# nanoporetech/pomfret

Hardware: AMD Instinct MI355X
Metric: aligned reads/sec (methphase kernel) (higher is better)
Workload: dtype u32/f32

## Files before the change

### pomfret_amd/csrc/pf_load.hip

```cpp
#include <hip/hip_runtime.h>
#include <stdint.h>
#include "pf_device.h"
#include "pf_load.h"

#define DEV static __device__ __forceinline__
#define NT_C 2u
#ifndef PF_K0_SEQ_REREAD
#define PF_K0_SEQ_REREAD 0
#endif

#ifdef PF_K0_PROFILE
DEV unsigned long long k0_now() {
    unsigned long long t;
    __builtin_amdgcn_sched_barrier(0);
    asm volatile("s_memtime %0\n\ts_waitcnt lgkmcnt(0)" : "=s"(t) :: "memory");
    __builtin_amdgcn_sched_barrier(0);
    return t;
}
#define K0_STAMP(i) do { const unsigned long long t_ = k0_now(); \
    if (d->ctr && lane == 0) atomicAdd(&d->ctr[8 + (i)], t_ - k0_t); k0_t = t_; } while (0)
#define K0_T0 unsigned long long k0_t = k0_now()
#else
#define K0_STAMP(i) do { } while (0)
#define K0_T0 do { } while (0)
#endif
#define NT_G 4u
#ifndef PF_K0_NOINL
#define PF_K0_NOINL 0
#endif
#if PF_K0_NOINL & 1
#define DEV_HBM static __device__ __attribute__((noinline))
#else
#define DEV_HBM DEV
#endif
#if PF_K0_NOINL & 2
#define DEV_COLD static __device__ __attribute__((noinline))
#else
#define DEV_COLD DEV
#endif
#ifndef PF_K0_PLACE
#define PF_K0_PLACE 1
#endif
#ifndef PF_K0_WALK2
#define PF_K0_WALK2 1
#endif
#ifndef PF_K0_FUSEC
#define PF_K0_FUSEC 1
#endif
#ifndef PF_K0_PADFIX
#define PF_K0_PADFIX 1
#endif
#ifndef PF_K0_NBRARE
#define PF_K0_NBRARE 1
#endif
#ifndef PF_K0_RANKDPP
#define PF_K0_RANKDPP 1
#endif
#ifndef PF_K0_HDRFAST
#define PF_K0_HDRFAST 1
#endif
#ifndef PF_K0_EMITDPP
#define PF_K0_EMITDPP 1
#endif
#ifndef PF_K0_ROWSKIP
#define PF_K0_ROWSKIP 1
#endif
#ifndef PF_K0_TILE128
#define PF_K0_TILE128 1
#endif
#ifndef PF_K0_DIAG1
#define PF_K0_DIAG1 0
#endif
#if PF_K0_DIAG1
#define K0_DIAG1(d) ((d)->diag == 1u)
#else
#define K0_DIAG1(d) false
#endif
#ifndef PF_K0_WPE
#define PF_K0_WPE 8
#endif

DEV uint32_t uni(uint32_t x) { return (uint32_t)__builtin_amdgcn_readfirstlane((int)x); }
DEV uint64_t lanemask_lt(uint32_t lane) { return lane ? (~0ull >> (64 - lane)) : 0ull; }
DEV uint32_t popc(uint64_t m) { return (uint32_t)__popcll(m); }
DEV uint32_t below_cnt(uint64_t b) {
    return __builtin_amdgcn_mbcnt_hi((uint32_t)(b >> 32), __builtin_amdgcn_mbcnt_lo((uint32_t)b, 0u));
}
DEV uint32_t rdl(uint32_t x, uint32_t l) { return (uint32_t)__builtin_amdgcn_readlane((int)x, (int)l); }

#define K0_CONST __attribute__((address_space(4)))
typedef const K0_CONST pf_load_dev *K0Args;
typedef const K0_CONST pf_k0_hdr *K0HdrP;
DEV K0Args k0_args() { return (K0Args)__builtin_amdgcn_kernarg_segment_ptr(); }
template <typename P>
DEV P k0_late(P p) {
    asm volatile("" : "+s"(p));
    return p;
}

DEV void wsync() {
    __builtin_amdgcn_fence(__ATOMIC_RELEASE, "workgroup");
    __builtin_amdgcn_wave_barrier();
    __builtin_amdgcn_fence(__ATOMIC_ACQUIRE, "workgroup");
}

DEV uint32_t dpp_shr_add(uint32_t x, const int ctrl) {
    uint32_t y;
    switch (ctrl) {
    case 1: y = (uint32_t)__builtin_amdgcn_update_dpp(0, (int)x, 0x111, 0xF, 0xF, true); break;
    case 2: y = (uint32_t)__builtin_amdgcn_update_dpp(0, (int)x, 0x112, 0xF, 0xF, true); break;
    case 4: y = (uint32_t)__builtin_amdgcn_update_dpp(0, (int)x, 0x114, 0xF, 0xF, true); break;
    case 8: y = (uint32_t)__builtin_amdgcn_update_dpp(0, (int)x, 0x118, 0xF, 0xF, true); break;
    case 15: y = (uint32_t)__builtin_amdgcn_update_dpp(0, (int)x, 0x142, 0xA, 0xF, false); break;
    default: y = (uint32_t)__builtin_amdgcn_update_dpp(0, (int)x, 0x143, 0xC, 0xF, false); break;
    }
    return x + y;
}
DEV uint32_t wscan(uint32_t x, uint32_t) {
    x = dpp_shr_add(x, 1);
    x = dpp_shr_add(x, 2);
    x = dpp_shr_add(x, 4);
    x = dpp_shr_add(x, 8);
    x = dpp_shr_add(x, 15);
    x = dpp_shr_add(x, 31);
    return x;
}
DEV uint64_t wscan64(uint64_t x, uint32_t lane) {
#pragma unroll
    for (int o = 1; o < 64; o <<= 1) {
        const uint64_t y = __shfl_up(x, o, 64);
        if (lane >= (uint32_t)o) x += y;
    }
    return x;
}
DEV uint64_t rdl64(uint64_t x, uint32_t l) {
    return ((uint64_t)rdl((uint32_t)(x >> 32), l) << 32) | rdl((uint32_t)x, l);
}

DEV uint32_t nib(const uint8_t *s, uint32_t i) { return (s[i >> 1] >> ((~i & 1u) << 2)) & 0xFu; }
DEV uint32_t nibw(uint64_t w, uint32_t i) { return (uint32_t)(w >> (8u * (i >> 1) + ((i & 1u) ? 0u : 4u))) & 0xFu; }
DEV uint32_t match16(uint64_t w, uint32_t tb, uint32_t nv) {
    uint32_t m = 0;
#pragma unroll
    for (uint32_t i = 0; i < 16; i++) m |= (nibw(w, i) == tb && i < nv) ? (1u << i) : 0u;
    return m;
}
DEV uint32_t select_bit(uint32_t m, uint32_t k) {
    for (uint32_t i = 0; i < k; i++) m &= m - 1;
    return (uint32_t)__builtin_ctz(m);
}
DEV bool is_digit(uint32_t c) { return c >= '0' && c <= '9'; }
// ... 17 lines not shown
    uint8_t eC[PF_K0_EC];
    uint8_t mC[2 * PF_K0_EC];
};
struct K0Seq {
    uint16_t sb[8 * 64];
    uint8_t sc[8 * 64];
};
struct K0Wide {
    uint32_t E[128], Off[128];
    uint32_t gE[16], sE[4];
    uint8_t T[128];
    uint32_t mV[64];
    uint8_t mC[64];
};
struct K0W {
    uint32_t T[PF_K0_TCAP];
    union {
        struct {
            uint32_t opE[64], opOff[64], opA[64];
            uint8_t opT[64];
            union {
                K0Seq s;
                K0Merge mg;
            } u;
        };
        K0Wide w;
    };
};
static_assert(sizeof(K0W) == 5120, "K0W: 5 KB per wave, 20,480 B per block");

struct K0Out {
    uint32_t n, first, last;
    uint32_t sorted, lim;
    uint32_t *pos;
    uint8_t *cat;
};

struct K0Tgt { uint32_t nd, nc, mi, th, te; uint64_t ml; };
#define PF_K0_MAXT 8
#define PF_K0_TW 7
struct K0Tgts { K0Tgt t0; uint32_t n, over; uint32_t *xt; };
DEV void k0_tgt_put(uint32_t *xt, uint32_t e, const K0Tgt &t, uint32_t lane) {
    if (lane == 0) {
        uint32_t *q = xt + PF_K0_TW * (e - 1);
        q[0] = t.nd; q[1] = t.nc; q[2] = t.mi; q[3] = t.th; q[4] = t.te; q[5] = (uint32_t)t.ml;
        q[6] = (uint32_t)(t.ml >> 32);
    }
}
DEV K0Tgt k0_tgt_get(const K0Tgts &T, uint32_t e) {
    if (e == 0) return T.t0;
    const uint32_t *q = T.xt + PF_K0_TW * (e - 1);
    K0Tgt t;
    t.nd = q[0]; t.nc = q[1]; t.mi = q[2]; t.th = q[3]; t.te = q[4];
    t.ml = ((uint64_t)q[6] << 32) | q[5];
    return t;
}

DEV uint32_t bytes_eq(uint32_t w, uint32_t c) {
    const uint32_t t = w ^ (c * 0x01010101u);
    return ~(((t & 0x7F7F7F7Fu) + 0x7F7F7F7Fu) | t) & 0x80808080u;
}
DEV uint32_t bytes_in(int32_t b, uint32_t lo, uint32_t hi) {
    const int32_t s = min(max((int32_t)lo - b, 0), 4), e = min(max((int32_t)hi - b, 0), 4);
    const uint32_t ml = s >= 4 ? 0u : 0x80808080u << (8 * s);
    const uint32_t mh = e <= 0 ? 0u : 0x80808080u >> (8 * (4 - e));
    return ml & mh;
}
DEV uint32_t wsum_small(uint32_t c) {
    return popc(__ballot(c & 1u)) + 2u * popc(__ballot(c & 2u)) + 4u * popc(__ballot(c & 4u));
}
DEV uint64_t nondigit_bytes(uint64_t y) {
    const uint64_t hi = (y & 0xF0F0F0F0F0F0F0F0ull) ^ 0x3030303030303030ull;
    const uint64_t hz = ~(((hi & 0x7F7F7F7F7F7F7F7Full) + 0x7F7F7F7F7F7F7F7Full) | hi) & 0x8080808080808080ull;
    const uint64_t ge10 = ((y & 0x0F0F0F0F0F0F0F0Full) + 0x7676767676767676ull) & 0x8080808080808080ull;
    return (~hz & 0x8080808080808080ull) | ge10;
}
DEV uint32_t swar_dec(uint64_t y, uint32_t n) {
    uint64_t z = (y & ((1ull << (8 * n)) - 1)) << (8 * (8 - n));
    z = ((z & 0x0F0F0F0F0F0F0F0Full) * 2561u) >> 8;
    z = ((z & 0x00FF00FF00FF00FFull) * 6553601u) >> 16;
    return (uint32_t)(((z & 0x0000FFFF0000FFFFull) * 42949672960001ull) >> 32);
}

struct K0Hdr { uint32_t base, strand, nc, h; int mi; };

template <bool MULTI>
DEV bool k0_mm_entries(const uint32_t *gw, const uint8_t *mm, uint32_t mis, uint32_t mlen, uint32_t mln,
                       uint32_t lane, K0Tgts &T) {
    T.n = 0;
    T.over = 0;
    T.t0.nd = 0;
    if (mlen == 0) return true;
    const uint32_t wend = mis + mlen;
    const uint32_t kmaxw = (wend - 1) / 4 + 1;
    auto ld = [&](uint32_t k) { return gw[min(k, kmaxw)]; };
    uint32_t k0 = 0;
    uint32_t w = ld(lane), pw = ld(64 + lane), pw2 = ld(128 + lane), pw3 = ld(192 + lane);
    auto byte_at = [&](uint32_t x) -> uint32_t {
        const uint32_t kx = (mis + x) >> 2, sh = 8 * ((mis + x) & 3u);
        if (kx - k0 < 64) return (rdl(w, kx - k0) >> sh) & 0xFFu;
        if (kx - k0 < 128) return (rdl(pw, kx - k0 - 64) >> sh) & 0xFFu;
        return mm[x];
    };
    K0Hdr H;
#if PF_K0_HDRFAST
    auto dword_at = [&](uint32_t kx) -> uint32_t {
        if (kx - k0 < 64) return rdl(w, kx - k0);
        if (kx - k0 < 128) return rdl(pw, kx - k0 - 64);
        return gw[min(kx, kmaxw)];
    };
#endif
    auto header = [&](uint32_t i) {
#if PF_K0_HDRFAST
        if (i + 3 < mlen) {
            const uint32_t x = mis + i, kx = x >> 2, sh = 8u * (x & 3u);
            const uint32_t lo = dword_at(kx);
            const uint32_t b4 = sh ? (lo >> sh) | (dword_at(kx + 1) << (32u - sh)) : lo;
            const uint32_t c2 = (b4 >> 16) & 0xFFu, c3 = b4 >> 24;
            if (is_alpha(c2) && !is_alpha(c3)) {
                H.base = b4 & 0xFFu;
                H.strand = (b4 >> 8) & 0xFFu;
                H.nc = 1;
                H.mi = c2 == 'm' ? 0 : -1;
                H.h = i + 3 + ((c3 == '.' || c3 == '?') ? 1u : 0u);
                return;
            }
        }
#endif
        H.base = byte_at(i);
        H.strand = i + 1 < mlen ? byte_at(i + 1) : 0u;
        uint32_t h = i + 2, nc = 0;
        int mi = -1;
        uint32_t c = h < mlen ? byte_at(h) : 0u;
        if (is_digit(c)) {
            while (h < mlen && is_digit(byte_at(h))) h++;
            nc = 1;
        } else {
            while (h < mlen && is_alpha(c = byte_at(h))) {
                if (c == 'm' && mi < 0) mi = (int)nc;
                nc++;
                h++;
            }
        }
        if (h < mlen && ((c = byte_at(h)) == '.' || c == '?')) h++;
        H.h = h; H.nc = nc; H.mi = mi;
    };
    uint64_t ml_cur = 0;
    auto close = [&](uint32_t i, uint32_t e, uint32_t commas) -> bool {
        if (e - i < 3) return false;
        if (H.strand != '+' && H.strand != '-') return false;
        if (H.nc == 0) return false;
        if (H.base == ',') commas--;
        if (H.base == 'C' && H.mi >= 0 && commas > 0) {
            if (mln && ml_cur + (uint64_t)commas * H.nc > mln) return false;
            if (!MULTI && T.n) { T.n = 2; return true; }
            if (T.n == PF_K0_MAXT) { T.over = 1; return true; }
            K0Tgt t;
            t.nd = commas; t.nc = H.nc; t.mi = (uint32_t)H.mi; t.th = H.h; t.te = e; t.ml = ml_cur;
            if (T.n == 0) T.t0 = t;
            else if constexpr (MULTI) k0_tgt_put(T.xt, T.n, t, lane);
            T.n++;
        }
        ml_cur += (uint64_t)commas * H.nc;
        return true;
    };
    uint32_t i = 0, ci = 0, cg = 0;
    header(0);
    for (;;) {
        const int32_t b = (int32_t)(4 * (k0 + lane)) - (int32_t)mis;
        const uint32_t vm = bytes_in(b, 0, mlen);
        const uint32_t sm = bytes_eq(w, ';') & vm, cm = bytes_eq(w, ',') & vm;
        const uint32_t ncl = (uint32_t)__builtin_popcount(cm);
        const uint32_t cin = wscan(ncl, lane);
        for (uint64_t bs = __ballot(sm != 0); bs; bs &= bs - 1) {
            const uint32_t l0 = (uint32_t)__ffsll((long long)bs) - 1;
            const uint32_t sml = rdl(sm, l0), cml = rdl(cm, l0), cb0 = cg + rdl(cin, l0) - rdl(ncl, l0);
            for (uint32_t m = sml; m; m &= m - 1) {
                const uint32_t sb = (uint32_t)__builtin_ctz(m) >> 3;
                const uint32_t e = 4 * (k0 + l0) - mis + sb;
                const uint32_t ce = cb0 + (uint32_t)__builtin_popcount(cml & ((1u << (8 * sb)) - 1u));
                if (!close(i, e, ce - ci)) return false;
                i = e + 1;
                ci = ce;
                if (i < mlen) header(i);
            }
        }
        cg += rdl(cin, 63);
        if (4 * (k0 + 64) >= wend) break;
        k0 += 64;
        w = pw;
        pw = pw2;
        pw2 = pw3;
        pw3 = ld(k0 + 192 + lane);
    }
    if (i < mlen && !close(i, mlen, cg - ci)) return false;
    if (mln && ml_cur > mln) return false;
    return true;
}

DEV uint32_t nondigit4(uint32_t y) {
    const uint32_t hi = (y & 0xF0F0F0F0u) ^ 0x30303030u;
    const uint32_t hz = ~(((hi & 0x7F7F7F7Fu) + 0x7F7F7F7Fu) | hi) & 0x80808080u;
    const uint32_t ge10 = ((y & 0x0F0F0F0Fu) + 0x76767676u) & 0x80808080u;
    return (~hz & 0x80808080u) | ge10;
}
DEV uint32_t pack4(uint32_t f) {
    uint32_t x = f >> 7;
    x |= x >> 7;
    x |= x >> 14;
    return x & 0xFu;
}
DEV uint32_t k0_dw(uint32_t i) {
    const uint32_t e = i & 7u;
    return (i >> 3) * ((e & 1u) ? 10u : 1u) * ((e & 2u) ? 100u : 1u) * ((e & 4u) ? 10000u : 1u);
}
DEV void k0_dw_table(uint32_t *tbl, uint32_t lane) {
    tbl[lane] = k0_dw(lane);
    if (lane < 16u) tbl[64u + lane] = k0_dw(64u + lane);
}

template <typename TP>
DEV_COLD bool k0_mm_ranks_swar(const uint32_t *gw, const uint8_t *mm, uint32_t mis, const K0Tgt &t, bool rev, TP TB,
                          uint32_t lane);

template <typename TP>
DEV bool k0_mm_ranks(const uint32_t *gw, const uint8_t *mm, uint32_t mis, const K0Tgt &t, bool rev, TP TB,
                     const uint32_t *tbl, uint32_t lane) {
    if (mm[t.th] != ',') return false;
    const uint32_t lo = t.th;
    uint32_t hi = t.te;
    const uint32_t wend = mis + t.te;
    uint64_t carry = 0;
    uint32_t kk = 0;
    const uint32_t k0s = (mis + lo) >> 2;
    const uint32_t kmaxw = (wend - 1) / 4 + 2;
    auto ld = [&](uint32_t k) { return gw[min(k, kmaxw)]; };
#if PF_K0_RANKDPP
    uint32_t w = ld(k0s + lane), pw = ld(k0s + lane + 64);
    uint32_t nd0 = pack4(nondigit4(w));
#else
    uint32_t w = ld(k0s + lane), wn = ld(k0s + lane + 1), wn2 = ld(k0s + lane + 2);
#endif
    for (uint32_t k0 = k0s; 4 * k0 < wend; k0 += 64) {
        const uint32_t k = k0 + lane;
#if PF_K0_RANKDPP
        const uint32_t ppw = ld(k + 128);
        const uint32_t ndn = pack4(nondigit4(pw));
        const uint32_t nd1 = (uint32_t)__builtin_amdgcn_update_dpp((int)rdl(ndn, 0), (int)nd0, 0x130, 0xF, 0xF, false);
        const uint32_t nd2 = (uint32_t)__builtin_amdgcn_update_dpp((int)rdl(ndn, 1), (int)nd1, 0x130, 0xF, 0xF, false);
        const uint32_t ndm = nd0 | (nd1 << 4) | (nd2 << 8);
#else
        const uint32_t pw = ld(k + 64), pwn = ld(k + 65), pwn2 = ld(k + 66);
        const uint32_t ndm = pack4(nondigit4(w)) | (pack4(nondigit4(wn)) << 4) | (pack4(nondigit4(wn2)) << 8);
#endif
        const int32_t b = (int32_t)(4 * k) - (int32_t)mis;
        const uint32_t nlo = (uint32_t)min(max((int32_t)lo - b, 0), 4);
        const uint32_t cw = pack4(bytes_eq(w, ','));
        uint32_t M, vb, cb;
        for (;;) {
            const uint32_t nin = (uint32_t)min(max((int32_t)hi - b, 0), 12);
            M = ndm | (~0u << nin);
            vb = (0xFu << nlo) & ~(~0u << min(nin, 4u)) & 0xFu;
            cb = cw & vb;
            const uint32_t jb = vb & M & ~cb;
            const uint64_t bj = __ballot(jb != 0);
            if (!bj) break;
            const uint32_t l0 = (uint32_t)__ffsll((long long)bj) - 1;
            hi = rdl((uint32_t)(b + (int32_t)__builtin_ctz(jb | 0x10u)), l0);
        }
        const uint32_t D = ~M & 0xFFFu;
        uint32_t x8 = D & (D >> 1);
        x8 &= x8 >> 2;
        x8 &= x8 >> 4;
        const uint32_t db = D & vb;
        const bool badc = (cb & (M >> 1)) != 0;
        if (__ballot((x8 & db) != 0 || badc)) {
            if (__ballot((x8 & db) != 0)) return k0_mm_ranks_swar(gw, mm, mis, t, rev, TB, lane);
            return false;
        }
        uint32_t c[4];
#pragma unroll
        for (uint32_t j = 0; j < 4; j++) {
            const uint32_t e = ((uint32_t)__builtin_ctz(M >> j) - 1u) & 7u;
            const uint32_t ix = ((db >> j) & 1u) ? ((((w >> (8 * j)) & 0xFu) << 3) | e) : 0u;
            c[j] = tbl[ix];
        }
        const uint32_t p1 = c[0], p2 = p1 + c[1], p3 = p2 + c[2], ls = p3 + c[3];
        const uint32_t nc = (uint32_t)__builtin_popcount(cb);
        const uint32_t sincl = wscan(ls, lane), cincl = wscan(nc, lane);
        const uint64_t part = carry + (sincl - ls);
        const uint32_t kl = kk + cincl - nc;
        auto pre = [&](uint32_t j) { return j == 0 ? 0u : j == 1 ? p1 : j == 2 ? p2 : p3; };
        bool ovf = false;
        if (nc > 0 && kl > 0) {
            const uint64_t rank = part + pre((uint32_t)__builtin_ctz(cb)) + (kl - 1);
            ovf |= rank > 0xFFFFFFFFull;
            TB[rev ? t.nd - kl : kl - 1] = (uint32_t)rank;
        }
        if (nc > 1) {
            const uint64_t rank = part + pre((uint32_t)__builtin_ctz(cb & (cb - 1))) + kl;
            ovf |= rank > 0xFFFFFFFFull;
            TB[rev ? t.nd - 1 - kl : kl] = (uint32_t)rank;
        }
        if (__ballot(ovf)) return false;
        carry += (uint64_t)rdl(sincl, 63);
        kk += rdl(cincl, 63);
#if PF_K0_RANKDPP
        w = pw; pw = ppw; nd0 = ndn;
#else
        w = pw; wn = pwn; wn2 = pwn2;
#endif
    }
    if (kk != t.nd) return false;
    const uint64_t last = carry + (t.nd - 1);
    if (last > 0xFFFFFFFFull) return false;
    if (lane == 0) TB[rev ? 0u : t.nd - 1] = (uint32_t)last;
    return true;
}

template <typename TP>
DEV_COLD bool k0_mm_ranks_swar(const uint32_t *gw, const uint8_t *mm, uint32_t mis, const K0Tgt &t, bool rev, TP TB,
                     uint32_t lane) {
    if (mm[t.th] != ',') return false;
    const uint32_t wend = mis + t.te;
    uint64_t carry = 0;
    uint32_t idx = 0;
    bool bad = false;
    for (uint32_t k0 = (mis + t.th) >> 2; 4 * k0 < wend; k0 += 64) {
        const uint32_t k = k0 + lane;
        const int32_t b = (int32_t)(4 * k) - (int32_t)mis;
        const uint32_t w = 4 * k < wend ? gw[k] : 0u;
        const uint32_t wn = 4 * k + 4 < wend ? gw[k + 1] : 0u;
        const uint32_t cm = bytes_eq(w, ',') & bytes_in(b, t.th, t.te);
        const uint32_t nl = (uint32_t)__builtin_popcount(cm);
        const uint32_t ie = wscan(nl, lane);
        const uint32_t gi0 = idx + ie - nl;
        const uint64_t x = ((uint64_t)wn << 32) | w;
        uint32_t vq[4] = {0, 0, 0, 0};
        uint64_t lsum = 0;
        bool ok = true;
        uint32_t m = cm;
#pragma unroll
        for (uint32_t q = 0; q < 4; q++) {
            if (!__ballot(q < nl)) break;
            if (q < nl) {
                const uint32_t pb = (uint32_t)__builtin_ctz(m) >> 3;
                m &= m - 1;
                const uint32_t xc = (uint32_t)(b + (int32_t)pb);
                const uint32_t win = 7 - pb, lim = t.te - xc - 1;
                const uint64_t y = x >> (8 * (pb + 1));
                const uint32_t n = (uint32_t)__builtin_ctzll(nondigit_bytes(y)) >> 3;
                const bool last = gi0 + q + 1 >= t.nd;
                uint64_t v;
                if (n < win || lim <= win) {
                    const uint32_t nv = n < lim ? n : lim;
                    v = nv ? swar_dec(y, nv) : 0u;
                    ok = ok && nv > 0;
                    if (!last) ok = ok && nv < lim && (uint32_t)((y >> (8 * nv)) & 0xFFu) == ',';
                } else {
                    uint32_t kk = xc + 1;
                    v = 0;
                    while (kk < t.te && is_digit(mm[kk])) { v = v * 10u + (uint64_t)(mm[kk] - '0'); kk++; }
                    ok = ok && v <= 0xFFFFFFFFull;
                    if (!last) ok = ok && kk < t.te && mm[kk] == ',';
                }
                vq[q] = (uint32_t)v;
                lsum += (uint32_t)v;
            }
        }
        const uint64_t incl = (__ballot(lsum >= (1ull << 24)) ? wscan64(lsum, lane) : (uint64_t)wscan((uint32_t)lsum, lane)) +
                              carry;
        uint64_t run = incl - lsum;
#pragma unroll
        for (uint32_t q = 0; q < 4; q++) {
// ... 787 lines not shown
template <typename TP>
DEV bool k0_merge_targets(K0Args d, K0W &L, const K0Tgts &T, uint32_t N, bool rev, TP TB,
                          const uint32_t *gw, const uint8_t *mmg, uint32_t mis, const uint8_t *ml, uint32_t mln,
                          uint32_t lane, uint32_t &nd_out, bool &past, bool &ovf) {
    nd_out = 0;
    ovf = false;
    unsigned long long t0 = 0;
    if (lane == 0) t0 = atomicAdd(d->stage_ctr, 2ull * N);
    const uint64_t cb = d->stage_off[d->n_recs] + (((uint64_t)uni((uint32_t)(t0 >> 32)) << 32) | uni((uint32_t)t0));
    if (cb + 2ull * N > d->stage_cap) {
        if (lane == 0) atomicOr(d->status, PF_ST_STAGE_OVF);
        ovf = true;
        return false;
    }
    uint32_t *tmp = d->stage_pos + cb, *mrg = tmp + N;
    k0_dw_table(L.u.mg.mV, lane);
    wsync();
    bool pst = false;
    for (uint32_t e = 0, oe = 0; e < T.n; e++) {
        const K0Tgt te = k0_tgt_get(T, e);
        uint32_t *TBe = tmp + oe;
        if (!k0_mm_ranks(gw, mmg, mis, te, rev, TBe, L.u.mg.mV, lane)) return false;
        wsync();
        for (uint32_t j = lane; j < te.nd; j += 64) {
            const uint32_t q = mln ? (uint32_t)ml[te.ml + (uint64_t)j * te.nc + te.mi] : 255u;
            const uint32_t sj = rev ? te.nd - 1 - j : j;
            const uint32_t rk = TBe[sj];
            pst |= rk >= (1u << 24);
            TBe[sj] = (rk & 0xFFFFFFu) | (q << 24);
        }
        wsync();
        oe += te.nd;
    }
    past = __ballot(pst) != 0;
    if (past) return true;
    for (uint32_t e = 0, oe = 0; e < T.n; e++) {
        const uint32_t ne = k0_tgt_get(T, e).nd;
        for (uint32_t j = lane; j < ne; j += 64) {
            const uint32_t v = tmp[oe + (rev ? ne - 1 - j : j)], rk = v & 0xFFFFFFu;
            uint32_t pos = j;
            for (uint32_t f = 0, of = 0; f < T.n; f++) {
                const uint32_t nf = k0_tgt_get(T, f).nd;
                if (f != e) {
                    uint32_t lo = 0, hi = nf;
                    while (lo < hi) {
                        const uint32_t mid = (lo + hi) >> 1;
                        const uint32_t x = tmp[of + (rev ? nf - 1 - mid : mid)] & 0xFFFFFFu;
                        if (f < e ? x <= rk : x < rk) lo = mid + 1;
                        else hi = mid;
                    }
                    pos += lo;
                }
                of += nf;
            }
            mrg[pos] = v;
        }
        oe += ne;
    }
    wsync();
    uint32_t kept = 0;
    for (uint32_t k0 = 0; k0 < N; k0 += 64) {
        const uint32_t k = k0 + lane;
        const bool keep = k < N && (k + 1 == N || (mrg[k] & 0xFFFFFFu) != (mrg[k + 1] & 0xFFFFFFu));
        kept += popc(__ballot(keep));
    }
    for (uint32_t k0 = 0, base = 0; k0 < N; k0 += 64) {
        const uint32_t k = k0 + lane;
        const uint32_t v = k < N ? mrg[k] : 0u;
        const bool keep = k < N && (k + 1 == N || (v & 0xFFFFFFu) != (mrg[k + 1] & 0xFFFFFFu));
        const uint64_t b = __ballot(keep);
        if (keep) {
            const uint32_t j = base + popc(b & lanemask_lt(lane));
            TB[rev ? kept - 1 - j : j] = v;
        }
        base += popc(b);
    }
    wsync();
    nd_out = kept;
    return true;
}

template <bool MULTI, typename TP>
DEV void k0_record(K0Args d, K0W &L, K0HdrP h, uint32_t lane, TP TB, uint32_t cap, const K0Tgts &T,
                   bool okm) {
    K0Tgt t = T.t0;
    bool multi = false;
    uint32_t ndsum = t.nd;
    if constexpr (MULTI) {
        multi = T.n > 1;
        for (uint32_t e = 1; e < T.n; e++) ndsum += k0_tgt_get(T, e).nd;
    }
    const bool rev = (h->flag_mapq & 16u) != 0;
    const uint8_t *mmg = d->mm + h->mm_off;
    const uint8_t *ml = d->ml + h->ml_off;
    const uint32_t mln = h->ml_len;

    bool okmm = okm;
    uint32_t nT = 0, mlq0 = 0xFFFFFFFFu, mlq1 = 0xFFFFFFFFu;
    bool implicit = false;
    K0_T0;
    {
        const uint32_t mis = (uint32_t)(reinterpret_cast<uintptr_t>(mmg) & 3u);
        const uint32_t *gw = reinterpret_cast<const uint32_t *>(mmg - mis);
        if (okmm && ndsum > cap) okmm = false;
        if (okmm && t.nd && !multi) {
            if (mln) {
                uint32_t q[8];
#pragma unroll
                for (uint32_t u = 0; u < 8; u++) {
                    const uint32_t j = min(lane + 64u * u, t.nd - 1);
                    q[u] = ml[t.ml + (uint64_t)j * t.nc + t.mi];
                }
                mlq0 = q[0] | (q[1] << 8) | (q[2] << 16) | (q[3] << 24);
                mlq1 = q[4] | (q[5] << 8) | (q[6] << 16) | (q[7] << 24);
            }
            k0_dw_table(L.u.mg.mV, lane);
            wsync();
            okmm = k0_mm_ranks(gw, mmg, mis, t, rev, TB, L.u.mg.mV, lane);
        }
    }
    wsync();
    bool past = false;
    if constexpr (MULTI) {
        if (okmm && multi) {
            if (d->ctr && lane == 0) atomicAdd(&d->ctr[PF_K0C_MULTICM], 1ull);
            bool ovf = false;
            uint32_t ndm = 0;
            const uint32_t mis = (uint32_t)(reinterpret_cast<uintptr_t>(mmg) & 3u);
            okmm = k0_merge_targets(d, L, T, ndsum, rev, TB, reinterpret_cast<const uint32_t *>(mmg - mis), mmg, mis,
                                    ml, mln, lane, ndm, past, ovf);
            if (ovf) { if (lane == 0) d->rec_n[h->rec] = PF_NONE; return; }
            t.nd = ndm;
        }
    }
    if (!multi && okmm && t.nd) {
        uint32_t u = 0;
        for (uint32_t j = lane; j < t.nd; j += 64, u++) {
            const uint32_t q = !mln ? 255u : u < 8 ? ((u < 4 ? mlq0 : mlq1) >> (8 * (u & 3))) & 0xFFu
                                                   : (uint32_t)ml[t.ml + (uint64_t)j * t.nc + t.mi];
            const uint32_t sj = rev ? t.nd - 1 - j : j;
            const uint32_t rk = TB[sj];
            past |= rk >= (1u << 24);
            TB[sj] = (rk & 0xFFFFFFu) | (q << 24);
        }
        past = __ballot(past) != 0;
        wsync();
    }
    K0_STAMP(0);
    d = k0_late(d);
    h = k0_late(h);
    if (d->diag == 2u) { if (lane == 0) d->rec_n[h->rec] = PF_NONE; return; }
    const uint8_t *seq = d->seq + h->seq_off;
    const uint32_t len = h->l_qseq;
    uint32_t tb_off = 0;
    if (okmm && t.nd && !past) nT = k0_seq_pass(d, L, seq, len, rev, t, TB, lane, implicit, tb_off);
    TB = TB + uni(tb_off);
    K0_STAMP(1);
    d = k0_late(d);
    h = k0_late(h);
    const uint32_t r = h->rec;
    if (d->diag == 3u || d->diag == 5u) { if (lane == 0) d->rec_n[r] = PF_NONE; return; }
    const uint32_t ncig = h->ncig;
    const uint32_t *cig = d->cigar + h->cig_off;
    if (!okmm && d->ctr && lane == 0) atomicAdd(&d->ctr[PF_K0C_BADMM], 1ull);
    nT = uni(nT);

    if (ncig == 0 || nT == 0) {
        if (lane == 0) d->rec_n[r] = PF_NONE;
        return;
    }
    uint64_t cb = h->stage_off;
    if (implicit || nT > h->stage_len) {
        const uint64_t need = (uint64_t)nT + (uint64_t)(len + 1) / 2;
        unsigned long long t = 0;
        if (lane == 0) t = atomicAdd(d->stage_ctr, (unsigned long long)need);
        cb = d->stage_off[d->n_recs] + (((uint64_t)uni((uint32_t)(t >> 32)) << 32) | uni((uint32_t)t));
        if (cb + need > d->stage_cap) {
            if (lane == 0) { atomicOr(d->status, PF_ST_STAGE_OVF); d->rec_n[r] = PF_NONE; }
            return;
        }
    }
    K0Out o;
    o.n = 0; o.first = 0; o.last = 0; o.sorted = 1; o.lim = 0;
    o.pos = d->stage_pos + cb;
    o.cat = d->stage_cat + cb;
    if (implicit && d->ctr && lane == 0) atomicAdd(&d->ctr[PF_K0C_IMPLICIT], 1ull);

    const uint32_t qs = h->pos;
    const bool stale = (cig[0] & 15u) == 4u && (TB[nT - 1] >> 2) <= (cig[0] >> 4);
    bool fatal = false, walked = false;
    uint32_t racc = 0;
    if (stale || d->force_seq) {
        if (d->ctr && lane == 0) atomicAdd(&d->ctr[PF_K0C_SEQPATH], 1ull);
        K0Out s = o;
        bool f = false;
        if (lane == 0) k0_walk_seq<1>(cig, ncig, qs, rev, TB, nT, implicit ? seq : nullptr, len, s, f);
        k0_bcast(o, s);
        fatal = uni(f ? 1u : 0u) != 0;
    } else {
#if PF_K0_TILE128
        if (!implicit) fatal = !k0_walk128<1>(d, L, cig, ncig, qs, rev, TB, nT, lane, o, racc);
        else fatal = !k0_walk<1>(d, L, cig, ncig, qs, rev, TB, nT, seq, len, true, lane, o, racc);
#else
        fatal = !k0_walk<1>(d, L, cig, ncig, qs, rev, TB, nT, seq, len, implicit, lane, o, racc);
#endif
        walked = true;
    }
    K0_STAMP(2);
    if (fatal) {
        if (lane == 0) { atomicOr(d->status, PF_ST_FATAL_CIGAR); d->rec_n[r] = PF_NONE; }
        return;
    }
    if (o.lim && lane == 0) atomicOr(d->status, PF_ST_POS_LIMIT);
    if (!o.sorted && o.n > 1) {
        if (d->ctr && lane == 0) atomicAdd(&d->ctr[PF_K0C_UNSORTED], 1ull);
        __builtin_amdgcn_fence(__ATOMIC_RELEASE, "agent");
        if (lane == 0) {
            for (uint32_t i = 1; i < o.n; i++) {
                const uint32_t v = o.pos[i];
                const uint8_t cc = o.cat[i];
                uint32_t k = i;
                while (k > 0 && (o.pos[k - 1] > v || (o.pos[k - 1] == v && o.cat[k - 1] > cc))) {
                    o.pos[k] = o.pos[k - 1];
                    o.cat[k] = o.cat[k - 1];
                    k--;
                }
                o.pos[k] = v;
                o.cat[k] = cc;
            }
        }
    }
    uint32_t rlen = racc;
    if (!walked)
        for (uint32_t c = lane; c < ncig; c += 64) rlen += k0_refc(cig[c]);
    rlen = rdl(wscan(rlen, lane), 63);
    if (lane < 8) {
        const uint32_t v = lane == 0 ? qs : lane == 1 ? qs + rlen : lane == 2 ? o.first : lane == 3 ? o.last
                         : lane == 4 ? (uint32_t)cb : lane == 5 ? (uint32_t)(cb >> 32) : 0u;
        d->rec_out[8ull * r + lane] = v;
    }
    if (lane == 63) {
        d->rec_n[r] = o.n;
        const uint32_t w = h->rec_win;
        atomicAdd(&d->win_kept[w], 1u);
        atomicAdd(&d->win_calls[w], o.n);
    }
    K0_STAMP(3);
}

template <bool MULTI>
DEV_HBM void k0_record_hbm(K0Args d, K0W &L, K0HdrP h, uint32_t lane, const K0Tgts &T, bool okm) {
    k0_record<MULTI>(d, L, h, lane, d->scr + h->scr_off, h->scr_len, T, okm);
}

template <bool MULTI>
DEV void k0_one(K0Args d, K0W &L, uint32_t slot, uint32_t lane) {
    const K0HdrP h = k0_rec(d, slot);
    const uint32_t fm = h->flag_mapq, flag = fm & 0xFFFFu, len = h->l_qseq;
    const bool drop = (flag & 4u) || (flag & 256u) || (flag & 2048u) || (fm >> 16) < d->min_mapq ||
                      len < 2u || len < d->min_len || (double)h->de > 0.1;
    if (drop) {
        if (lane == 0) d->rec_n[h->rec] = PF_NONE;
        return;
    }
    if (d->diag == 4u) { if (lane == 0) d->rec_n[h->rec] = PF_NONE; return; }
    const uint8_t *mmg = d->mm + h->mm_off;
    const uint32_t mis = (uint32_t)(reinterpret_cast<uintptr_t>(mmg) & 3u);
    K0Tgts T;
    T.xt = L.opE;
    const bool okm = k0_mm_entries<MULTI>(reinterpret_cast<const uint32_t *>(mmg - mis), mmg, mis, h->mm_len, h->ml_len, lane, T);
    if (T.over) {
        if (lane == 0) { atomicOr(d->status, PF_ST_MM_LIMIT); d->rec_n[h->rec] = PF_NONE; }
        return;
    }
    if (!MULTI && okm && T.n > 1) {
        if (lane == 0) d->multi_list[atomicAdd(d->multi_ctr, 1u)] = slot;
        return;
    }
    uint32_t ndsum = T.t0.nd;
    if constexpr (MULTI)
        for (uint32_t e = 1; e < T.n; e++) ndsum += k0_tgt_get(T, e).nd;
    if (h->scr_len == 0 || !okm || uni(ndsum) <= (uint32_t)PF_K0_TCAP)
        k0_record<MULTI>(d, L, h, lane, L.T, (uint32_t)PF_K0_TCAP, T, okm);
    else k0_record_hbm<MULTI>(d, L, h, lane, T, okm);
}

__global__ __launch_bounds__(PF_K0_WAVES * 64) __attribute__((amdgpu_waves_per_eu(PF_K0_WPE))) void pf_k0_load(pf_load_dev) {
    __shared__ K0W lds[PF_K0_WAVES];
    const K0Args d = k0_args();
    const uint32_t lane = threadIdx.x & 63u;
    const uint32_t wv = uni(threadIdx.x >> 6);
    const uint32_t slot = blockIdx.x * PF_K0_WAVES + wv;
    if (slot >= d->n_recs) return;
    k0_one<false>(d, lds[wv], slot, lane);
}

__global__ __launch_bounds__(PF_K0_WAVES * 64) void pf_k0_multi(pf_load_dev) {
    __shared__ K0W lds[PF_K0_WAVES];
    const K0Args d = k0_args();
    const uint32_t lane = threadIdx.x & 63u;
    const uint32_t wv = uni(threadIdx.x >> 6);
    const uint32_t n = *d->multi_ctr;
    for (uint32_t i = blockIdx.x * PF_K0_WAVES + wv; i < n; i += gridDim.x * PF_K0_WAVES)
        k0_one<true>(d, lds[wv], d->multi_list[i], lane);
}

template <uint32_t NT, typename T>
DEV T blk_excl_scan(T v, T *sh, T &total) {
    static_assert(NT % 64 == 0 && NT <= 4096, "block of whole waves");
    const uint32_t tid = threadIdx.x, lane = tid & 63u, wid = tid >> 6;
    constexpr uint32_t NW = NT / 64;
    T x = v;
#pragma unroll
    for (int o = 1; o < 64; o <<= 1) {
        const T y = __shfl_up(x, o, 64);
        if (lane >= (uint32_t)o) x += y;
    }
    if (lane == 63) sh[wid] = x;
    __syncthreads();
    if (wid == 0) {
        T s = lane < NW ? sh[lane] : (T)0;
#pragma unroll
        for (int o = 1; o < 64; o <<= 1) {
            const T y = __shfl_up(s, o, 64);
            if (lane >= (uint32_t)o) s += y;
        }
        if (lane < NW) sh[NW + lane] = s;
    }
    __syncthreads();
    const T base = wid ? sh[NW + wid - 1] : (T)0;
    total = sh[2 * NW - 1];
    __syncthreads();
    return base + x - v;
}

__global__ __launch_bounds__(PF_SCAN_THREADS) void pf_k0_scan(pf_load_dev d) {
    __shared__ uint64_t sh[2 * (PF_SCAN_THREADS / 64)];
    __shared__ uint32_t sh32[2 * (PF_SCAN_THREADS / 64)];
    const uint32_t tid = threadIdx.x, W = d.n_windows;
    uint32_t rc = 0;
    uint64_t cc = 0, sc = 0;
    for (uint32_t w0 = 0; w0 < W; w0 += PF_SCAN_THREADS) {
        const uint32_t w = w0 + tid;
        const uint32_t kept = w < W ? d.win_kept[w] : 0u;
        const uint64_t calls = w < W ? (uint64_t)d.win_calls[w] : 0ull;
        const int32_t sel = w < W ? max(d.win_par[4ull * w], 1) : 1;
        const uint64_t slots = w < W ? calls / (2ull * (uint64_t)sel) + 1ull : 0ull;
        uint32_t tk;
        uint64_t tcl, ts;
        const uint32_t ek = blk_excl_scan<PF_SCAN_THREADS, uint32_t>(kept, sh32, tk);
        const uint64_t ec = blk_excl_scan<PF_SCAN_THREADS, uint64_t>(calls, sh, tcl);
        const uint64_t es = blk_excl_scan<PF_SCAN_THREADS, uint64_t>(slots, sh, ts);
        if (w < W) {
            d.win_read_off[w] = rc + ek;
            d.win_call_off[w] = cc + ec;
            d.win_site_off[w] = sc + es;
            d.win_site_cap[w] = (uint32_t)min(slots, (uint64_t)0xFFFFFFF0u);
        }
        rc += tk;
        cc += tcl;
        sc += ts;
    }
    const uint32_t st = __hip_atomic_load(d.status, __ATOMIC_RELAXED, __HIP_MEMORY_SCOPE_AGENT);
    const bool s_ovf = sc > d.sites_cap;
    const bool empty = s_ovf || (st & (PF_ST_STAGE_OVF | PF_ST_FATAL_CIGAR | PF_ST_POS_LIMIT));
    if (tid == 0) {
// ... 65 lines not shown
```

Measured before the change: 61.88 million.

## Add single-pass MM rank computation and fast full-row paths in MM parsing

Adds an optional mode (PF_K0_MMONCE, off by default) that computes methylation ranks while scanning MM entries, so the separate k0_mm_ranks pass can be skipped. With PF_K0_MMROWS on by default, it also adds fast paths: rows lying fully inside the MM string skip the per-byte validity mask, and a row with no semicolons uses a cheaper ballot-based sum in place of a wave scan. In k0_mm_ranks, interior rows skip the boundary-adjustment loop and a no-overflow row takes a simplified rank store. The cost is extra branching and more register pressure in the hot loops.

```diff
diff --git a/pomfret_amd/csrc/pf_load.hip b/pomfret_amd/csrc/pf_load.hip
--- a/pomfret_amd/csrc/pf_load.hip
+++ b/pomfret_amd/csrc/pf_load.hip
@@ -67,6 +67,12 @@
 #endif
 #ifndef PF_K0_TILE128
 #define PF_K0_TILE128 1
+#endif
+#ifndef PF_K0_MMONCE
+#define PF_K0_MMONCE 0
+#endif
+#ifndef PF_K0_MMROWS
+#define PF_K0_MMROWS 1
 #endif
 #ifndef PF_K0_DIAG1
 #define PF_K0_DIAG1 0
@@ -250,15 +256,50 @@
     return (uint32_t)(((z & 0x0000FFFF0000FFFFull) * 42949672960001ull) >> 32);
 }
 
+DEV uint32_t nondigit4(uint32_t y) {
+    const uint32_t hi = (y & 0xF0F0F0F0u) ^ 0x30303030u;
+    const uint32_t hz = ~(((hi & 0x7F7F7F7Fu) + 0x7F7F7F7Fu) | hi) & 0x80808080u;
+    const uint32_t ge10 = ((y & 0x0F0F0F0Fu) + 0x76767676u) & 0x80808080u;
+    return (~hz & 0x80808080u) | ge10;
+}
+DEV uint32_t pack4(uint32_t f) {
+    uint32_t x = f >> 7;
+    x |= x >> 7;
+    x |= x >> 14;
+    return x & 0xFu;
+}
+DEV uint32_t k0_rank_first(uint32_t part, uint32_t cb, const uint32_t (&c)[4]) {
+    const uint32_t bl = (cb & (0u - cb)) - 1u;
+    return part + ((bl & 1u) ? c[0] : 0u) + ((bl & 2u) ? c[1] : 0u) + ((bl & 4u) ? c[2] : 0u);
+}
+DEV uint32_t k0_rank_second(uint32_t part, uint32_t cb, const uint32_t (&c)[4]) {
+    return part + c[0] + c[1] + ((cb & 8u) ? c[2] : 0u);
+}
+DEV uint32_t k0_dw(uint32_t i) {
+    const uint32_t e = i & 7u;
+    return (i >> 3) * ((e & 1u) ? 10u : 1u) * ((e & 2u) ? 100u : 1u) * ((e & 4u) ? 10000u : 1u);
+}
+DEV void k0_dw_table(uint32_t *tbl, uint32_t lane) {
+    tbl[lane] = k0_dw(lane);
+    if (lane < 16u) tbl[64u + lane] = k0_dw(64u + lane);
+}
+
 struct K0Hdr { uint32_t base, strand, nc, h; int mi; };
-
-template <bool MULTI>
+struct K0True { static constexpr bool value = true; };
+struct K0False { static constexpr bool value = false; };
+
+template <bool MULTI, bool RANK>
 DEV bool k0_mm_entries(const uint32_t *gw, const uint8_t *mm, uint32_t mis, uint32_t mlen, uint32_t mln,
-                       uint32_t lane, K0Tgts &T) {
+                       uint32_t lane, K0Tgts &T, uint32_t *TB, uint32_t *tbl, bool &ranked) {
     T.n = 0;
     T.over = 0;
     T.t0.nd = 0;
+    ranked = false;
     if (mlen == 0) return true;
+    if constexpr (RANK) {
+        k0_dw_table(tbl, lane);
+        wsync();
+    }
     const uint32_t wend = mis + mlen;
     const uint32_t kmaxw = (wend - 1) / 4 + 1;
     auto ld = [&](uint32_t k) { return gw[min(k, kmaxw)]; };
@@ -333,27 +374,101 @@
         return true;
     };
     uint32_t i = 0, ci = 0, cg = 0;
+    bool rk = false;
+    uint32_t rth = 0, rsum = 0;
+    uint32_t ndc = 0, ndk = ~0u;
+    auto rank_open = [&]() {
+        rk = T.n == 0 && H.base == 'C' && H.mi >= 0 && H.h < mlen && byte_at(H.h) == ',';
+        rth = H.h;
+        rsum = 0;
+    };
+    auto rank_close = [&]() {
+        const uint64_t last = (uint64_t)rsum + (T.t0.nd - 1);
+        ranked = rk && last <= 0xFFFFFFFFull;
+        if (ranked && lane == 0 && T.t0.nd <= (uint32_t)PF_K0_TCAP) TB[T.t0.nd - 1] = (uint32_t)last;
+    };
     header(0);
+    if constexpr (RANK) rank_open();
     for (;;) {
         const int32_t b = (int32_t)(4 * (k0 + lane)) - (int32_t)mis;
-        const uint32_t vm = bytes_in(b, 0, mlen);
+        const uint32_t vm = PF_K0_MMROWS && 4 * k0 >= mis && 4 * (k0 + 64) <= wend ? 0x80808080u : bytes_in(b, 0, mlen);
         const uint32_t sm = bytes_eq(w, ';') & vm, cm = bytes_eq(w, ',') & vm;
         const uint32_t ncl = (uint32_t)__builtin_popcount(cm);
-        const uint32_t cin = wscan(ncl, lane);
-        for (uint64_t bs = __ballot(sm != 0); bs; bs &= bs - 1) {
+        const uint64_t bs0 = __ballot(sm != 0);
+        uint32_t cin = 0, ctot;
+        if (!PF_K0_MMROWS || bs0 || rk) {
+            cin = wscan(ncl, lane);
+            ctot = rdl(cin, 63);
+        } else ctot = wsum_small(ncl);
+        auto rank_row = [&](uint32_t hi, auto full) {
+            constexpr bool FULL = decltype(full)::value;
+            uint32_t nd0 = ndc;
+            if (ndk != k0) nd0 = pack4(nondigit4(w));
+            const uint32_t ndn = pack4(nondigit4(pw));
+            ndc = ndn;
+            ndk = k0 + 64;
+            const uint32_t nd1 = (uint32_t)__builtin_amdgcn_update_dpp((int)rdl(ndn, 0), (int)nd0, 0x130, 0xF, 0xF, false);
+            const uint32_t nd2 = (uint32_t)__builtin_amdgcn_update_dpp((int)rdl(ndn, 1), (int)nd1, 0x130, 0xF, 0xF, false);
+            const uint32_t nlo = FULL ? 0u : (uint32_t)min(max((int32_t)rth - b, 0), 4);
+            const uint32_t nin = FULL ? 12u : (uint32_t)min(max((int32_t)hi - b, 0), 12);
+            const uint32_t M = nd0 | (nd1 << 4) | (nd2 << 8) | (~0u << nin);
+            const uint32_t vb = FULL ? 0xFu : (0xFu << nlo) & ~(~0u << min(nin, 4u)) & 0xFu;
+            const uint32_t cw = pack4(cm);
+            const uint32_t cb = cw & vb;
+            const uint32_t D = ~M & 0xFFFu;
+            uint32_t x8 = D & (D >> 1);
+            x8 &= x8 >> 2;
+            x8 &= x8 >> 4;
+            const uint32_t db = D & vb;
+            if (__ballot(((vb & M & ~cb) | (cb & (M >> 1)) | (x8 & db)) != 0)) { rk = false; return; }
+            uint32_t c[4];
+#pragma unroll
+            for (uint32_t j = 0; j < 4; j++) {
+                const uint32_t e = ((uint32_t)__builtin_ctz(M >> j) - 1u) & 7u;
+                const uint32_t ix = ((db >> j) & 1u) ? ((((w >> (8 * j)) & 0xFu) << 3) | e) : 0u;
+                c[j] = tbl[ix];
+            }
+            const uint32_t ls = c[0] + c[1] + c[2] + c[3];
+            const uint32_t nc = (uint32_t)__builtin_popcount(cb);
+            const uint32_t sincl = wscan(ls, lane);
+            if ((uint64_t)rsum + rdl(sincl, 63) + (cg + ctot - ci) > 0xFFFFFFFFull) { rk = false; return; }
+            const uint32_t part = rsum + (sincl - ls);
+            const uint32_t kl = cg + cin - ncl - ci + (FULL ? 0u : (uint32_t)__builtin_popcount(cw & ~(0xFu << nlo)));
+            const uint32_t r1 = k0_rank_first(part, cb, c) + (kl - 1), r2 = k0_rank_second(part, cb, c) + kl;
+            if (nc > 0 && kl > 0 && kl - 1 < (uint32_t)PF_K0_TCAP) TB[kl - 1] = r1;
+            if (nc > 1 && kl < (uint32_t)PF_K0_TCAP) TB[kl] = r2;
+            rsum += rdl(sincl, 63);
+        };
+        for (uint64_t bs = bs0; bs; bs &= bs - 1) {
             const uint32_t l0 = (uint32_t)__ffsll((long long)bs) - 1;
             const uint32_t sml = rdl(sm, l0), cml = rdl(cm, l0), cb0 = cg + rdl(cin, l0) - rdl(ncl, l0);
             for (uint32_t m = sml; m; m &= m - 1) {
                 const uint32_t sb = (uint32_t)__builtin_ctz(m) >> 3;
                 const uint32_t e = 4 * (k0 + l0) - mis + sb;
                 const uint32_t ce = cb0 + (uint32_t)__builtin_popcount(cml & ((1u << (8 * sb)) - 1u));
+                if constexpr (RANK) {
+                    if (rk) rank_row(e, K0False());
+                }
+                const uint32_t tn = T.n;
                 if (!close(i, e, ce - ci)) return false;
+                if constexpr (RANK) {
+                    if (tn == 0 && T.n == 1) rank_close();
+                }
                 i = e + 1;
                 ci = ce;
-                if (i < mlen) header(i);
-            }
-        }
-        cg += rdl(cin, 63);
+                if (i < mlen) {
+                    header(i);
+                    if constexpr (RANK) rank_open();
+                } else rk = false;
+            }
+        }
+        if constexpr (RANK) {
+            if (rk) {
+                if ((int32_t)rth <= (int32_t)(4 * k0) - (int32_t)mis && 4 * (k0 + 64) + 8 <= wend) rank_row(mlen, K0True());
+                else rank_row(mlen, K0False());
+            }
+        }
+        cg += ctot;
         if (4 * (k0 + 64) >= wend) break;
         k0 += 64;
         w = pw;
@@ -361,30 +476,15 @@
         pw2 = pw3;
         pw3 = ld(k0 + 192 + lane);
     }
-    if (i < mlen && !close(i, mlen, cg - ci)) return false;
+    if (i < mlen) {
+        const uint32_t tn = T.n;
+        if (!close(i, mlen, cg - ci)) return false;
+        if constexpr (RANK) {
+            if (tn == 0 && T.n == 1) rank_close();
+        }
+    }
     if (mln && ml_cur > mln) return false;
     return true;
-}
-
-DEV uint32_t nondigit4(uint32_t y) {
-    const uint32_t hi = (y & 0xF0F0F0F0u) ^ 0x30303030u;
-    const uint32_t hz = ~(((hi & 0x7F7F7F7Fu) + 0x7F7F7F7Fu) | hi) & 0x80808080u;
-    const uint32_t ge10 = ((y & 0x0F0F0F0Fu) + 0x76767676u) & 0x80808080u;
-    return (~hz & 0x80808080u) | ge10;
-}
-DEV uint32_t pack4(uint32_t f) {
-    uint32_t x = f >> 7;
-    x |= x >> 7;
-    x |= x >> 14;
-    return x & 0xFu;
-}
-DEV uint32_t k0_dw(uint32_t i) {
-    const uint32_t e = i & 7u;
-    return (i >> 3) * ((e & 1u) ? 10u : 1u) * ((e & 2u) ? 100u : 1u) * ((e & 4u) ? 10000u : 1u);
-}
-DEV void k0_dw_table(uint32_t *tbl, uint32_t lane) {
-    tbl[lane] = k0_dw(lane);
-    if (lane < 16u) tbl[64u + lane] = k0_dw(64u + lane);
 }
 
 template <typename TP>
@@ -422,19 +522,28 @@
         const uint32_t ndm = pack4(nondigit4(w)) | (pack4(nondigit4(wn)) << 4) | (pack4(nondigit4(wn2)) << 8);
 #endif
         const int32_t b = (int32_t)(4 * k) - (int32_t)mis;
-        const uint32_t nlo = (uint32_t)min(max((int32_t)lo - b, 0), 4);
         const uint32_t cw = pack4(bytes_eq(w, ','));
         uint32_t M, vb, cb;
-        for (;;) {
-            const uint32_t nin = (uint32_t)min(max((int32_t)hi - b, 0), 12);
-            M = ndm | (~0u << nin);
-            vb = (0xFu << nlo) & ~(~0u << min(nin, 4u)) & 0xFu;
-            cb = cw & vb;
-            const uint32_t jb = vb & M & ~cb;
-            const uint64_t bj = __ballot(jb != 0);
-            if (!bj) break;
-            const uint32_t l0 = (uint32_t)__ffsll((long long)bj) - 1;
-            hi = rdl((uint32_t)(b + (int32_t)__builtin_ctz(jb | 0x10u)), l0);
+        bool inner = PF_K0_MMROWS && (int32_t)lo <= (int32_t)(4 * k0) - (int32_t)mis && 4 * (k0 + 64) + 8 <= mis + hi;
+        if (inner) {
+            M = ndm | 0xFFFFF000u;
+            vb = 0xFu;
+            cb = cw;
+            if (__ballot((M & ~cb & 0xFu) != 0)) inner = false;
+        }
+        if (!inner) {
+            const uint32_t nlo = (uint32_t)min(max((int32_t)lo - b, 0), 4);
+            for (;;) {
+                const uint32_t nin = (uint32_t)min(max((int32_t)hi - b, 0), 12);
+                M = ndm | (~0u << nin);
+                vb = (0xFu << nlo) & ~(~0u << min(nin, 4u)) & 0xFu;
+                cb = cw & vb;
+                const uint32_t jb = vb & M & ~cb;
+                const uint64_t bj = __ballot(jb != 0);
+                if (!bj) break;
+                const uint32_t l0 = (uint32_t)__ffsll((long long)bj) - 1;
+                hi = rdl((uint32_t)(b + (int32_t)__builtin_ctz(jb | 0x10u)), l0);
+            }
         }
         const uint32_t D = ~M & 0xFFFu;
         uint32_t x8 = D & (D >> 1);
@@ -456,8 +565,22 @@
         const uint32_t p1 = c[0], p2 = p1 + c[1], p3 = p2 + c[2], ls = p3 + c[3];
         const uint32_t nc = (uint32_t)__builtin_popcount(cb);
         const uint32_t sincl = wscan(ls, lane), cincl = wscan(nc, lane);
+        const uint32_t kl = kk + cincl - nc;
+        if (PF_K0_MMROWS && carry + rdl(sincl, 63) + kk + rdl(cincl, 63) <= 0xFFFFFFFFull) {
+            const uint32_t r1 = k0_rank_first((uint32_t)carry + (sincl - ls), cb, c) + (kl - 1);
+            const uint32_t r2 = k0_rank_second((uint32_t)carry + (sincl - ls), cb, c) + kl;
+            if (nc > 0 && kl > 0) TB[rev ? t.nd - kl : kl - 1] = r1;
+            if (nc > 1) TB[rev ? t.nd - 1 - kl : kl] = r2;
+            carry += (uint64_t)rdl(sincl, 63);
+            kk += rdl(cincl, 63);
+#if PF_K0_RANKDPP
+            w = pw; pw = ppw; nd0 = ndn;
+#else
+            w = pw; wn = pwn; wn2 = pwn2;
+#endif
+            continue;
+        }
         const uint64_t part = carry + (sincl - ls);
-        const uint32_t kl = kk + cincl - nc;
         auto pre = [&](uint32_t j) { return j == 0 ? 0u : j == 1 ? p1 : j == 2 ? p2 : p3; };
         bool ovf = false;
         if (nc > 0 && kl > 0) {
@@ -1411,7 +1534,7 @@
 
 template <bool MULTI, typename TP>
 DEV void k0_record(K0Args d, K0W &L, K0HdrP h, uint32_t lane, TP TB, uint32_t cap, const K0Tgts &T,
-                   bool okm) {
+                   bool okm, bool ranked) {
     K0Tgt t = T.t0;
     bool multi = false;
     uint32_t ndsum = t.nd;
@@ -1443,9 +1566,20 @@
                 mlq0 = q[0] | (q[1] << 8) | (q[2] << 16) | (q[3] << 24);
                 mlq1 = q[4] | (q[5] << 8) | (q[6] << 16) | (q[7] << 24);
             }
-            k0_dw_table(L.u.mg.mV, lane);
-            wsync();
-            okmm = k0_mm_ranks(gw, mmg, mis, t, rev, TB, L.u.mg.mV, lane);
+            if (ranked) {
+                if (rev) {
+                    wsync();
+                    for (uint32_t j = lane; j < t.nd / 2; j += 64) {
+                        const uint32_t a = TB[j], b = TB[t.nd - 1 - j];
+                        TB[j] = b;
+                        TB[t.nd - 1 - j] = a;
+                    }
+                }
+            } else {
+                k0_dw_table(L.u.mg.mV, lane);
+                wsync();
+                okmm = k0_mm_ranks(gw, mmg, mis, t, rev, TB, L.u.mg.mV, lane);
+            }
         }
     }
     wsync();
@@ -1579,7 +1713,7 @@
 
 template <bool MULTI>
 DEV_HBM void k0_record_hbm(K0Args d, K0W &L, K0HdrP h, uint32_t lane, const K0Tgts &T, bool okm) {
-    k0_record<MULTI>(d, L, h, lane, d->scr + h->scr_off, h->scr_len, T, okm);
+    k0_record<MULTI>(d, L, h, lane, d->scr + h->scr_off, h->scr_len, T, okm, false);
 }
 
 template <bool MULTI>
@@ -1597,7 +1731,10 @@
     const uint32_t mis = (uint32_t)(reinterpret_cast<uintptr_t>(mmg) & 3u);
     K0Tgts T;
     T.xt = L.opE;
-    const bool okm = k0_mm_entries<MULTI>(reinterpret_cast<const uint32_t *>(mmg - mis), mmg, mis, h->mm_len, h->ml_len, lane, T);
+    constexpr bool ONCE = PF_K0_MMONCE && !MULTI;
+    bool ranked = false;
+    const bool okm = k0_mm_entries<MULTI, ONCE>(reinterpret_cast<const uint32_t *>(mmg - mis), mmg, mis, h->mm_len,
+                                                h->ml_len, lane, T, L.T, L.u.mg.mV, ranked);
     if (T.over) {
         if (lane == 0) { atomicOr(d->status, PF_ST_MM_LIMIT); d->rec_n[h->rec] = PF_NONE; }
         return;
@@ -1610,7 +1747,7 @@
     if constexpr (MULTI)
         for (uint32_t e = 1; e < T.n; e++) ndsum += k0_tgt_get(T, e).nd;
     if (h->scr_len == 0 || !okm || uni(ndsum) <= (uint32_t)PF_K0_TCAP)
-        k0_record<MULTI>(d, L, h, lane, L.T, (uint32_t)PF_K0_TCAP, T, okm);
+        k0_record<MULTI>(d, L, h, lane, L.T, (uint32_t)PF_K0_TCAP, T, okm, ONCE && ranked);
     else k0_record_hbm<MULTI>(d, L, h, lane, T, okm);
 }
 
```

Result: no change. 62.42 million (median of 6 runs) (+0.9%).
